# bwohlberg/sporco

Hardware: AMD Instinct MI355X
Metric: ConvBPDN ADMM iterations/s (higher is better)
Workload: dtype f32; 1 GPU; admm.cbpdn.ConvBPDN 512x512 greyscale, K=64 8x8 filters, N=32 images per GPU, lambda=0.05, default options (AutoRho, stats every iteration); global_images=32, parallelism=image-shard x1

## Files before the change

### include/sporco_amd.h

```cpp
#ifndef SPORCO_AMD_H
#define SPORCO_AMD_H

#include <stddef.h>
#include <stdint.h>

#ifdef __cplusplus
extern "C" {
#endif

#define SPORCO_AMD_F32 0
#define SPORCO_AMD_F64 1

#define SPORCO_AMD_OK 0
#define SPORCO_AMD_EINVAL (-1)
#define SPORCO_AMD_EHIP (-2)
#define SPORCO_AMD_ENOMEM (-3)
#define SPORCO_AMD_ESTATE (-4)


const char *sporco_amd_version(void);
const char *sporco_amd_last_error(void);
int sporco_amd_device_count(int *count);
int sporco_amd_device_info(int device, char *name, size_t name_len, int *cu_count,
                           size_t *hbm_bytes);
// ... 34 lines not shown
#define SPORCO_AMD_VAR_DMU0 22
#define SPORCO_AMD_VAR_WML 23
#define SPORCO_AMD_VAR_WMS 24
#define SPORCO_AMD_VAR_DX 32
#define SPORCO_AMD_VAR_DXF 33
#define SPORCO_AMD_VAR_DYF 34
#define SPORCO_AMD_VAR_DXFPRV 35
#define SPORCO_AMD_VAR_DYFPRV 36
#define SPORCO_AMD_VAR_DVF 37
#define SPORCO_AMD_VAR_DGF 38
#define SPORCO_AMD_VAR_DT0 39
#define SPORCO_AMD_VAR_DT1 40
#define SPORCO_AMD_VAR_DT2 41
#define SPORCO_AMD_VAR_DSX 42
#define SPORCO_AMD_VAR_DSU 43
#define SPORCO_AMD_VAR_COUNT 44

int sporco_amd_csc_create(const sporco_amd_dims *dims, int device, void *stream,
                          sporco_amd_csc_t *out);
int sporco_amd_csc_create_mc(const sporco_amd_dims *dims, int32_t dict_channels, int device,
                             void *stream, sporco_amd_csc_t *out);
int sporco_amd_csc_create_volume(const sporco_amd_dims *dims, int32_t depth, int device, void *stream,
                                 sporco_amd_csc_t *out);
int sporco_amd_csc_destroy(sporco_amd_csc_t h);
int sporco_amd_csc_sync(sporco_amd_csc_t h);
int sporco_amd_csc_stream(sporco_amd_csc_t h, void **stream);
#define SPORCO_AMD_QUERY_FUSED_COLS 0
#define SPORCO_AMD_QUERY_FUSED_ROWS 1
#define SPORCO_AMD_QUERY_FUSED_PGM 2
#define SPORCO_AMD_QUERY_DEVICE_FILTERS 3
#define SPORCO_AMD_QUERY_VFORM_LIVE 4
#define SPORCO_AMD_QUERY_PERSIST_RUNS 5
#define SPORCO_AMD_QUERY_CCMOD_GROUPS 6
int sporco_amd_csc_query(sporco_amd_csc_t h, int what, int *out);
int sporco_amd_csc_placement_report(sporco_amd_csc_t h, char *buf, size_t cap);
#define SPORCO_AMD_HINT_KEEP_VFORM 0
#define SPORCO_AMD_HINT_ONE_LAUNCH 1
#define SPORCO_AMD_MODE_COMPLEX_PAIR 2
#define SPORCO_AMD_VOLUME_FILTER_DEPTH 3
int sporco_amd_csc_set_hint(sporco_amd_csc_t h, int what, int value);

int sporco_amd_csc_set_signal(sporco_amd_csc_t h, const void *S);

int sporco_amd_csc_set_dict(sporco_amd_csc_t h, const void *D, int32_t dH, int32_t dW);
int sporco_amd_csc_set_dict_imag(sporco_amd_csc_t h, const void *D_imag, int32_t dH, int32_t dW);

int sporco_amd_csc_set_l1_weight(sporco_amd_csc_t h, const void *w, const int64_t shape[5]);
int sporco_amd_csc_set_l21_weight(sporco_amd_csc_t h, const void *w, const int64_t shape[5]);
int sporco_amd_csc_set_grad_weight(sporco_amd_csc_t h, const void *w);
int sporco_amd_csc_set_filter_sizes(sporco_amd_csc_t h, const int32_t *fh, const int32_t *fw);
int sporco_amd_csc_set_ams_mask(sporco_amd_csc_t h, const void *w, const int64_t shape[5]);

int sporco_amd_csc_upload(sporco_amd_csc_t h, int var, const void *src);
int sporco_amd_csc_download(sporco_amd_csc_t h, int var, void *dst);
int sporco_amd_csc_device_ptr(sporco_amd_csc_t h, int var, void **ptr_dev);


#define SPORCO_AMD_FLAG_NONNEG (1u << 0)
#define SPORCO_AMD_FLAG_NOBNDRY (1u << 1)
#define SPORCO_AMD_FLAG_JOINT (1u << 2)
#define SPORCO_AMD_FLAG_RESID (1u << 3)
#define SPORCO_AMD_FLAG_OBJ (1u << 4)
#define SPORCO_AMD_FLAG_XRRS (1u << 5)
#define SPORCO_AMD_FLAG_GEVAL_Y (1u << 6)
#define SPORCO_AMD_FLAG_FEVAL_Y (1u << 7)
#define SPORCO_AMD_FLAG_KEEP_X (1u << 8)
// ... 238 lines not shown
```

### sporco_amd/_lib.py

```python

import ctypes
import os

import numpy as np

F32, F64 = 0, 1

VAR_Y, VAR_U, VAR_X, VAR_XF, VAR_DF, VAR_SF = 0, 1, 2, 3, 4, 5
VAR_YF, VAR_XFPRV, VAR_YFPRV, VAR_VF, VAR_GF, VAR_AX, VAR_YPREV = 6, 7, 8, 9, 10, 11, 12
VAR_T0, VAR_T1, VAR_T2, VAR_ZF = 13, 14, 15, 16
VAR_CX, VAR_CU = 17, 18
VAR_MY0, VAR_MU0 = 19, 20
VAR_DMY0, VAR_DMU0 = 21, 22
VAR_WML, VAR_WMS = 23, 24
VAR_DX, VAR_DXF, VAR_DYF, VAR_DXFPRV, VAR_DYFPRV = 32, 33, 34, 35, 36
VAR_DVF, VAR_DGF, VAR_DT0, VAR_DT1, VAR_DT2 = 37, 38, 39, 40, 41
VAR_DSX, VAR_DSU = 42, 43
DSTEP_ISM, DSTEP_CG = 0, 1

FLAG_NONNEG = 1 << 0
FLAG_NOBNDRY = 1 << 1
FLAG_JOINT = 1 << 2
FLAG_RESID = 1 << 3
FLAG_OBJ = 1 << 4
FLAG_XRRS = 1 << 5
FLAG_GEVAL_Y = 1 << 6
FLAG_FEVAL_Y = 1 << 7
FLAG_KEEP_X = 1 << 8
FLAG_NO_X = 1 << 9
FLAG_GRADREG = 1 << 10
FLAG_AMS = 1 << 11
FLAG_DMASK = 1 << 12
QUERY_FUSED_COLS, QUERY_FUSED_ROWS, QUERY_FUSED_PGM, QUERY_DEVICE_FILTERS, QUERY_VFORM_LIVE = 0, 1, 2, 3, 4
QUERY_PERSIST_RUNS = 5
QUERY_CCMOD_GROUPS = 6
HINT_KEEP_VFORM = 0
HINT_ONE_LAUNCH = 1
MODE_COMPLEX_PAIR = 2
VOLUME_FILTER_DEPTH = 3

OUT_R2, OUT_S2, OUT_AX2, OUT_Y2, OUT_U2 = 0, 1, 2, 3, 4
OUT_DFID, OUT_L1, OUT_L21 = 5, 6, 7
OUT_XRRS_D2, OUT_XRRS_AX2, OUT_XRRS_B2 = 8, 9, 10
OUT_RGR = 11
OUT_CNSTR = 12
OUT_CGIT, OUT_CGN = 13, 14
OUT_COUNT = 16

PGM_F, PGM_DFID, PGM_L1, PGM_HESS, PGM_RSDL, PGM_FY, PGM_LIN, PGM_DXY2 = range(8)

EXPORTS = (
    'sporco_amd_version', 'sporco_amd_last_error', 'sporco_amd_device_count',
    'sporco_amd_device_info', 'sporco_amd_csc_create', 'sporco_amd_csc_create_mc', 'sporco_amd_csc_create_volume',
    'sporco_amd_csc_destroy',
    'sporco_amd_csc_sync', 'sporco_amd_csc_stream', 'sporco_amd_csc_query', 'sporco_amd_csc_placement_report', 'sporco_amd_csc_set_hint', 'sporco_amd_csc_set_signal', 'sporco_amd_csc_set_dict', 'sporco_amd_csc_set_dict_imag',
    'sporco_amd_csc_set_l1_weight', 'sporco_amd_csc_set_l21_weight',
    'sporco_amd_csc_set_grad_weight', 'sporco_amd_csc_set_ams_mask',
    'sporco_amd_csc_upload', 'sporco_amd_csc_download', 'sporco_amd_csc_device_ptr',
    'sporco_amd_csc_admm_iter', 'sporco_amd_csc_admm_iter_dev', 'sporco_amd_csc_admm_run',
    'sporco_amd_csc_admm_xstep', 'sporco_amd_csc_admm_relax',
    'sporco_amd_csc_admm_ystep', 'sporco_amd_csc_admm_ustep',
    'sporco_amd_csc_admm_stats', 'sporco_amd_csc_scale_u',
    'sporco_amd_csc_reconstruct', 'sporco_amd_csc_dhs_absmax',
    'sporco_amd_csc_pgm_grad', 'sporco_amd_csc_pgm_eval', 'sporco_amd_csc_pgm_prox_step',
    'sporco_amd_csc_pgm_iter', 'sporco_amd_csc_pgm_commit',
    'sporco_amd_csc_lincomb', 'sporco_amd_csc_pair_stats', 'sporco_amd_csc_copy',
    'sporco_amd_csc_pgm_resid', 'sporco_amd_csc_pgm_resid_stats',
    'sporco_amd_csc_fft_var', 'sporco_amd_csc_ifft_var',
# ... 768 lines not shown
```

### sporco_amd/csrc/api_admm_run.inc

```
    bool admm_run_supported(const sporco_amd_admm_params &p) const {
        return !cplx && std::is_same<T, float>::value && rows_ok && mr_ok(p) && (fused || fused_slabs) && !fused_mc &&
               !tail_mode && !(p.flags & (F_XRRS | F_GRADREG | F_KEEP_X | F_FEVAL_Y)) &&
               (!(p.flags & F_JOINT) || joint_rows_ok(p)) && p.lmbda >= 0.0 && p.rho > 0.0 &&
               !std::getenv("SPORCO_AMD_HOST_LOOP");
    }

    bool persist_ok(const sporco_amd_admm_params &p, const sporco_amd_admm_ctrl &c, bool vf,
                    bool has_reduce) const {
        const bool off = sw.persist >= 0 ? sw.persist != 1 : !hint_one_launch;
        return !off && vf && !has_reduce && fused && !fused_slabs && Ks == K && run_always_emit &&
               admm_persist_supported<T>(H, W, K) && !wl1.ptr && c.max_iter >= 3 &&
               !(p.flags & (F_NOBNDRY | F_AMS | F_JOINT)) && admm_persist_resident<T>(H, W, K, CN);
    }
    PersistIterArgs<T> persist_iter_args(const sporco_amd_admm_params &p, const T *vin, T *vout,
                                         double *prow, double *pcol) {
        PersistIterArgs<T> a;
        cx<T> *Xf = cv(SPORCO_AMD_VAR_XF);
        a.fwd.y = a.fwd.u = nullptr;
        a.fwd.v = vin;
        a.fwd.flags = p.flags;
        a.fwd.C = C;
        a.fwd.N = N;
        a.fwd.dH = p.dH;
        a.fwd.dW = p.dW;
// ... 65 lines not shown
            pst_grid = grid;
        }
        AdmmPersistArgs<T> a;
        const int p0 = index0 & 1;
        a.iter[p0] = persist_iter_args(p, v_prev, v_other, part_rows, part_f);
        a.iter[p0 ^ 1] = persist_iter_args(p, v_other, v_prev, pst_part_rows, pst_part_f);
        a.blk = static_cast<PersistIterArgs<T> *>(pst_blk);
        a.ctl_blk = pst_ctl;
        a.ctl = ctl_dev;
        a.rec = reinterpret_cast<AdmmRecord *>(rec_ring) + index0;
        a.index0 = index0;
        a.max_iter = max_iter - index0;
        a.bar = pst_bar;
        a.n_row_tiles = (int)nrow;
        a.n_col_tiles = (int)ncol;
        a.want_dfid = (p.flags & F_OBJ) ? 1 : 0;
        a.want_sums = want_sums ? 1 : 0;
        a.dfid_scale = 1.0 / ((double)H * W);
        SA_HIP(hipMemsetAsync(pst_bar, 0, sizeof(unsigned) * kPersistBarWords, st));
        {
            ProfScope ps(prof, PS_PERSIST);
            launch_admm_persist<T>(st, a, grid);
        }
        unsigned bar[16];
        SA_HIP(hipMemcpyAsync(bar, pst_bar, sizeof(bar), hipMemcpyDeviceToHost, st));
        sync();
        if (bar[2]) throw Error(SPORCO_AMD_EHIP, "one-launch solve: a grid barrier did not complete");
        xf_tiled = true;
        ++pst_runs;
        return (int)bar[3];
    }

    int64_t enqueue_iter_ctl(const sporco_amd_admm_params &p, const T *vin = nullptr,
                             T *vout = nullptr) {
        T *Y = vin ? nullptr : static_cast<T *>(vars[SPORCO_AMD_VAR_Y]);
        T *U = vin ? nullptr : static_cast<T *>(vars[SPORCO_AMD_VAR_U]);
        cx<T> *Xf = cv(SPORCO_AMD_VAR_XF);
        {
            RowsFwdArgs<T> ra;
            ra.y = Y;
            ra.u = U;
            ra.v = vin;
            ra.flags = p.flags;
            ra.C = C;
            ra.N = N;
            if (vin) {
                ra.wl1 = wl1;
                ra.dH = p.dH;
                ra.dW = p.dW;
                ra.ams_bits = ams_bits_of(p);
                ra.ams_k = Ku - 1;
            }
            ra.s2 = T(1);
            ra.t = Xf;
            ra.Ks = Ks;
            ra.twA = twRows;
            ra.H = H;
            ra.W = W;
            ra.CN = CN;
            ra.K = K;
            ra.P = P;
            ra.ctl = ctl_dev;
            ProfScope ps(prof, vin ? PS_ROWS_FWD_V : PS_ROWS_FWD);
            launch_rows_fwd<T>(st, ra);
        }
        {
            FusedColsArgs<T> fa;
// ... 37 lines not shown
        pa.twW = planW.tw<T>();
        pa.y = Y;
        pa.u = U;
        pa.y_out = y_alt;
        pa.u_out = u_alt;
        pa.v_in = vin;
        pa.v_out = vout;
        pa.x = nullptr;
        pa.scale = T(1.0 / ((double)H * (double)W));
        pa.rlx = (T)p.rlx;
        pa.thr = T(0);
        pa.u_scale = T(1);
        pa.flags = p.flags;
        pa.H = H;
        pa.W = W;
        pa.C = C;
        pa.N = N;
        pa.K = K;
        pa.dH = p.dH;
        pa.dW = p.dW;
        pa.P = P;
        pa.wl1 = wl1;
        pa.Ks = Ks;
        pa.ams_bits = ams_bits_of(p);
        pa.ams_k = Ku - 1;
        pa.partials = part_rows;
        pa.ctl = ctl_dev;
        int64_t nt = 0;
        if (!run_always_emit) {
            ProfScope ps(prof, vin ? PS_ROWS_INV_POST_V : PS_ROWS_INV_POST);
            nt = launch_rows_inv_post<T>(st, pa);
        }
        pa.t_next = Xf;
        {
            ProfScope ps(prof, vin ? PS_ROWS_INV_POST_V_EMIT : PS_ROWS_INV_POST_EMIT);
            nt = launch_rows_inv_post<T>(st, pa);
        }
        if (!vout) {
            std::swap(vars[SPORCO_AMD_VAR_Y], reinterpret_cast<void *&>(y_alt));
            std::swap(vars[SPORCO_AMD_VAR_U], reinterpret_cast<void *&>(u_alt));
        }
        return nt;
    }

    int admm_run(const sporco_amd_admm_params &p, const sporco_amd_admm_ctrl &c,
                 sporco_amd_admm_record *records, double *rho_out, double *u_scale_out,
                 sporco_amd_reduce_fn reduce, void *user) override {
        require_ready();
        if (!admm_run_supported(p)) return -1;
        if (gv_live) ensure_yu();
        SA_REQUIRE(c.max_iter >= 0, "max_iter must not be negative");
        if (c.max_iter == 0) {
            *rho_out = p.rho;
            *u_scale_out = p.u_scale;
            return 0;
        }
        if (!y_alt) alloc_alt_pair();
        const bool nn = p.flags & F_NONNEG, jn = p.flags & F_JOINT;
        if (v_live && (!vform_ok(p) || !vform_same_opts(p))) ensure_yu();
        const bool vf = vform_ok(p) && (v_live || c.max_iter >= 4 || hint_vform);
        if (!vf) ensure_yu();
        const bool v_at_entry = v_live;
        T *const v_entry = v_cur;
        const T v_entry_thr = v_thr, v_entry_thr21 = v_thr21;
        if (!ctl_dev) SA_HIP(hipMalloc((void **)&ctl_dev, sizeof(AdmmCtl)));
        if (rec_cap < c.max_iter) {
// ... 17 lines not shown
        in.xi = c.rho_xi;
        in.mu21 = p.mu;
        in.k = c.k0;
        in.stable_run = stable_run;
        in.emitted = t_ready ? 1 : 0;
        in.is_f32 = 1;
        in.autorho = c.auto_rho;
        in.period = c.period > 0 ? c.period : 1;
        in.autoscaling = c.auto_scaling;
        in.stdres = c.std_residuals;
        in.need_resid = c.need_residuals;
        in.thr_prev = v_at_entry ? (float)v_entry_thr : 0.f;
        in.thr21_prev = v_at_entry ? (float)v_entry_thr21 : 0.f;
        in.no_speculation = sw.no_speculation ? 1 : 0;
        run_always_emit = !in.no_speculation && E <= ((int64_t)1 << 22);
        if (run_always_emit) in.no_speculation = 2;
        launch_admm_ctl_init(st, ctl_dev, in);
        SA_HIP(hipMemsetAsync(out_dev, 0, sizeof(double) * kOutSlots, st));
        const int ahead = c.lookahead > 0 ? c.lookahead : 3;
        int enq = 0, done = 0, stop_at = -1;
        int lag = std::getenv("SPORCO_AMD_RUN_LAG") ? std::atoi(std::getenv("SPORCO_AMD_RUN_LAG")) : 0;
        auto poll = [&](int upto, bool block) {
            while (done < upto && stop_at < 0) {
                if (rec_ring[done].seq != done + 1) {
                    if (!block) return;
                    if (hipStreamQuery(st) == hipSuccess && rec_ring[done].seq != done + 1)
                        throw Error(SPORCO_AMD_EHIP, "device-driven solve: record not written");
                    continue;
                }
                if (rec_ring[done].stop) stop_at = done;
                ++done;
            }
        };
        T *vb_in = v_at_entry ? v_entry : nullptr;
        T *const vb_first = vf ? (vb_in == y_alt ? u_alt : y_alt) : nullptr;
        auto enqueue_one = [&]() {
            T *vb_out = vf ? (vb_in == y_alt ? u_alt : y_alt) : nullptr;
            const int64_t nt = enqueue_iter_ctl(p, vb_in, vb_out);
            vb_in = vb_out;
            if (want_sums) {
                const int slots[7] = {SPORCO_AMD_OUT_R2, SPORCO_AMD_OUT_S2, SPORCO_AMD_OUT_AX2,
                                      SPORCO_AMD_OUT_Y2, SPORCO_AMD_OUT_U2, SPORCO_AMD_OUT_L1,
                                      SPORCO_AMD_OUT_L21};
                const double scales[7] = {1, 1, 1, 1, 1, 1, 1};
                const int fslots[2] = {SPORCO_AMD_OUT_DFID, SPORCO_AMD_OUT_RGR};
                const double fscales[2] = {1.0 / ((double)H * W), 1.0 / ((double)H * W)};
                const bool dfid = p.flags & F_OBJ;
                {
                    ProfScope ps(prof, PS_FINALIZE);
                    launch_finalize2(st, part_rows, (int)nt, 8, (p.flags & F_JOINT) ? 7 : 6, slots,
                                     scales, part_f, part_f_rows,
                                     1, dfid ? 1 : 0, fslots, fscales, out_dev);
                }
                if (reduce) reduce(user, out_dev);
                else if (comm_user) comm_reduce_sums(comm_user, out_dev, st);
            }
            launch_admm_ctl_update(st, ctl_dev, out_dev, rec_ring + enq, enq, true);
            ++enq;
        };
        const bool shard = reduce != nullptr || comm_user != nullptr;
        const int wlag = shard ? 0 : lag;
        if (persist_ok(p, c, vf, shard)) {
            enqueue_one();
            T *v0 = vb_in, *v1 = (v0 == y_alt) ? u_alt : y_alt;
            enq += run_persist(p, 1, c.max_iter, v0, v1, want_sums);
            if (c.need_residuals) poll(enq, false);
        }
        for (; enq < c.max_iter && stop_at < 0 && !persist_ok(p, c, vf, shard);) {
            enqueue_one();
            if (c.need_residuals) {
                poll(enq - lag, false);
                if (stop_at < 0 && enq - wlag - done > ahead) poll(enq - wlag - ahead, true);
            }
        }
        if (shard && want_sums && c.need_residuals) {
            if (stop_at < 0) poll(enq, true);
            if (stop_at >= 0)
                while (enq < c.max_iter && enq < stop_at + 1 + ahead) enqueue_one();
        }
        sync();
        poll(enq, false);
        const int n = stop_at >= 0 ? stop_at + 1 : enq;
        if (!vf && ((enq - n) & 1)) {
            std::swap(vars[SPORCO_AMD_VAR_Y], reinterpret_cast<void *&>(y_alt));
            std::swap(vars[SPORCO_AMD_VAR_U], reinterpret_cast<void *&>(u_alt));
        }
        if (vf) {
            T *other_first = vb_first == y_alt ? u_alt : y_alt;
            v_cur = ((n - 1) & 1) ? other_first : vb_first;
            v_thr = (T)(p.lmbda / rec_ring[n - 1].rho);
            v_thr21 = (T)(p.mu / rec_ring[n - 1].rho);
            if (n >= 2) {
                v_prev_kind = 2;
// ... 104 lines not shown
```

### sporco_amd/csrc/csc_api.hip

```cpp
#include "csc_impl.h"

#include <chrono>
#include <string>

namespace sporco_amd {

thread_local std::string g_last_error;
std::atomic<int64_t> g_xfer[4];
const char *kProfNames[PS_COUNT] = {"fft_r2c_rows",     "fft_c2c_cols_fwd", "sm_solve",
                                           "fft_c2c_cols_inv", "fft_c2r_rows",     "admm_post",
                                           "fused_cols_sm",    "rows_fwd",         "rows_inv_post",
                                           "rows_inv_post_emit",
                                           "rows_fwd_v",       "rows_inv_post_v",  "rows_inv_post_v_emit",
                                           "pgm_grad_ifft",    "pgm_rows_prox",    "pgm_fft_momentum",
                                           "finalize",         "pgm_elementwise",  "other",
                                           "admm_persist_run",
                                    "setcoef_rows",     "setcoef_cols",     "ccmod_grad_tiled",
                                    "fft_c2r_vpost",    "fft_c2r_vpost_emit",
                                    "inhib_update"};

struct Switches {
    bool unfused, old_rows, no_pad, no_vform, no_speculation, no_cols_sm, md_generic, cns_generic, cg_host,
        placement_off, placement_force;
    int persist;
// ... 99 lines not shown
    }
    cx<T> *twRows = nullptr;
    double *part_rows = nullptr;
    double *pst_part_rows = nullptr, *pst_part_f = nullptr;
    void *pst_blk = nullptr;
    AdmmCtl *pst_ctl = nullptr;
    unsigned *pst_bar = nullptr;
    int pst_grid = 0, pst_runs = 0;
    T *y_alt = nullptr, *u_alt = nullptr;
    bool x_stale = false, x_invalid = false;
    bool md_x_pending = false;
    bool prev_in_alt = false;
    bool v_live = false;
    T *v_cur = nullptr;
    T v_thr = T(0), v_prev_thr = T(0);
    T v_thr21 = T(0), v_prev_thr21 = T(0), vp_thr21 = T(0);
    bool v_nonneg = false, v_joint = false;
    uint32_t v_opts = 0;
    int v_dH = 1, v_dW = 1;
    int v_prev_kind = 0;
    bool vp_pending = false;
    T *vp_buf = nullptr, *vp_free = nullptr;
    T vp_thr = T(0);
    bool vp_nonneg = false;
    uint64_t touch_epoch = 0, fused_epoch = ~(uint64_t)0;
    bool gv_live = false, gv_nonneg = false;
    T gv_thr = T(0);
    uint64_t gen_epoch = ~(uint64_t)0;
    bool t_ready = false;
    int stable_run = 0;
    AdmmCtl *ctl_dev = nullptr;
    AdmmRecord *rec_ring = nullptr;
    int rec_cap = 0;
    CgCtl *cg_dev = nullptr;
    CgPinned *cg_pin = nullptr;
    sporco_amd_admm_params last_p;
    bool zf_tiled = false;
    cx<T> *gpart = nullptr;
    int ccmod_groups = 1;
    bool pgm_tiled = false, pgm_x_stale = false;
    sporco_amd_pgm_params last_pgm;
    double *part_pgm = nullptr, *part_pgm2 = nullptr;
    cx<T> *ccmod_r = nullptr;
    cx<T> *pgm_ey = nullptr;
    bool pgm_held = false;
    bool run_always_emit = false;
    T *ghh = nullptr, *ghw = nullptr, *wg = nullptr;
    bool have_wg = false;
    T *g1t = nullptr;
    bool g1_valid = false;
    double g1_rho = 0.0, g1_mu = 0.0;

    int padded_filters(int H_, int W_, int K_) const {
        if (K_ % 2 == 0 || sw.unfused || sw.no_pad)
            return K_;
        const bool cols = fused_cols_supported<T>(H_, K_ + 1) || fused_slabs_supported<T>(H_, K_ + 1);
        return (cols && rows_supported<T>(W_, K_ + 1)) ? K_ + 1 : K_;
    }

    Csc(const sporco_amd_dims &d, int dev, void *stream, int cd, int depth_ = 1) : dm(d), device(dev) {
        SA_REQUIRE(d.H >= 1 && d.W >= 1 && d.C >= 1 && d.N >= 1 && d.K >= 1,
                   "all dimensions must be >= 1");
        SA_REQUIRE(cd == 1 || cd == d.C,
                   "a multi-channel dictionary needs as many channels as the signal");
        SA_HIP(hipSetDevice(device));
        H = d.H;
// ... 137 lines not shown
        (void)hipStreamSynchronize(st);
        place_release_spares();
        inhib_release();
        big_free(gemit);
        if (part_vpost) (void)hipFree(part_vpost);
        big_free(cols_out[0]);
        big_free(cols_out[1]);
        for (hipEvent_t e : place_ev)
            if (e) (void)hipEventDestroy(e);
        for (auto &v : vars) big_free(v);
        big_free(y_alt);
        big_free(u_alt);
        big_free(work);
        y_alt = u_alt = nullptr;
        work = nullptr;
        for (void *p : {(void *)pst_part_rows, (void *)pst_part_f, pst_blk, (void *)pst_ctl, (void *)pst_bar,
                        (void *)cns_w, (void *)cns_sft, (void *)flt_h, (void *)flt_w,
                        (void *)zf_ch, (void *)zfv_buf, (void *)md_sft, (void *)md_coef, (void *)pgm_rx[0], (void *)pgm_rx[1]})
            if (p) (void)hipFree(p);
        for (void *p : {(void *)dft, (void *)sft, (void *)gramt, (void *)part_f, (void *)twA, (void *)twB,
                        (void *)twRows, (void *)part_rows, (void *)y_alt, (void *)u_alt, (void *)part_pgm, (void *)part_pgm2, (void *)ccmod_r, (void *)pgm_ey, (void *)gpart,
                        (void *)qpart, (void *)coop_flags, (void *)ghh, (void *)ghw, (void *)wg, (void *)g1t, (void *)ism_gam, (void *)ism_del, (void *)ism_mm, (void *)dft_mc, (void *)sft_mc, (void *)bt_mc, (void *)cns_f, (void *)cns_m, (void *)sft_eff, (void *)coef_t, (void *)ams_bits, (void *)gramz_t,
                        (void *)cns_yold, (void *)md_s, (void *)dism_gam, (void *)dism_del, (void *)dism_mm,
                        (void *)dwork, (void *)pcn_stats, (void *)work, (void *)innerb, (void *)gram, (void *)dpad, (void *)sreal,
                        (void *)wl1_buf, (void *)wl21_buf, (void *)wams_buf, (void *)wdat_buf, (void *)part_a, (void *)part_b, (void *)part_cs, (void *)df_im, (void *)pgm_es[0], (void *)pgm_es[1], (void *)pgm_es[2], (void *)pgm_es[3],
                        (void *)out_dev_own})
            if (p) (void)hipFree(p);
        if (out_pinned) (void)hipHostFree(out_pinned);
        if (coop_err) (void)hipHostFree(coop_err);
        if (rec_ring) (void)hipHostFree(rec_ring);
        if (cg_pin) (void)hipHostFree((void *)cg_pin);
        if (cg_dev) (void)hipFree(cg_dev);
        if (ctl_dev) (void)hipFree(ctl_dev);
        planW.destroy();
        planH.destroy();
        if (depth > 1) planD.destroy();
        if (own_stream) (void)hipStreamDestroy(st);
    }

    int64_t KD() const { return (int64_t)Cd * K; }
    static bool var_is_signal_real(int var) {
        return var >= SPORCO_AMD_VAR_MY0 && var <= SPORCO_AMD_VAR_DMU0;
    }
    size_t var_bytes(int var) const {
        if (var == SPORCO_AMD_VAR_SF) return sizeof(cx<T>) * npix * CNs;
        if (var_is_signal_real(var)) return sizeof(T) * (int64_t)H * W * CNs;
        if (var_is_dict_sized(var))
            return var_is_complex(var) ? sizeof(cx<T>) * npix * KD()
                                       : sizeof(T) * (int64_t)H * W * KD();
        if (var == SPORCO_AMD_VAR_CX || var == SPORCO_AMD_VAR_CU) return sizeof(T) * E * Cd;
        return var_is_complex(var) ? sizeof(cx<T>) * EF : sizeof(T) * E;
    }

    size_t var_alloc_bytes(int var) const {
        return var == SPORCO_AMD_VAR_XF ? sizeof(cx<T>) * (size_t)std::max(EF, EFt) : var_bytes(var);
    }
    void *var_ptr(int var) {
        SA_REQUIRE(var_is_valid(var), "unknown state variable id");
        if (var == SPORCO_AMD_VAR_Y || var == SPORCO_AMD_VAR_U) {
            ++touch_epoch;
            if (v_live || gv_live) ensure_yu();
        }
        if (!vars[var]) {
            const size_t nb = var_alloc_bytes(var);
            big_alloc(&vars[var], nb);
            SA_HIP(hipMemsetAsync(vars[var], 0, nb, st));
// ... 52 lines not shown
    bool cols_striped() const { return cols_out[0] != nullptr; }
    void alloc_cols_out() {
        if (cols_out[0] || !std::is_same<T, float>::value || !fused || fused_slabs || tail_mode || Ks != K || !rows_ok || mr)
            return;
        const size_t plane = sizeof(cx<T>) * (size_t)CN * H * K;
        const size_t be = plane * (size_t)((Wf + 1) / 2), bo = plane * (size_t)(Wf / 2);
        if (!placement_on(be)) return;
        void *p0 = nullptr;
        big_alloc(&p0, be);
        cols_out[0] = static_cast<cx<T> *>(p0);
        cols_out[1] = static_cast<cx<T> *>(place_alloc(bo, {{p0, be}}, "cols_out_odd"));
    }
    void alloc_alt_pair() {
        if (y_alt) return;
        (void)var_ptr(SPORCO_AMD_VAR_XF);
        place_var(SPORCO_AMD_VAR_XF, {SPORCO_AMD_VAR_Y, SPORCO_AMD_VAR_U}, "T");
        void *t = vars[SPORCO_AMD_VAR_XF];
        const size_t tb = var_alloc_bytes(SPORCO_AMD_VAR_XF), nb = sizeof(T) * (size_t)E;
        y_alt = static_cast<T *>(place_alloc(nb, {{t, tb}}, "V0"));
        u_alt = static_cast<T *>(place_alloc(nb, {{t, tb}}, "V1"));
        place_var(SPORCO_AMD_VAR_Y, {SPORCO_AMD_VAR_XF}, "Y");
        place_var(SPORCO_AMD_VAR_U, {SPORCO_AMD_VAR_XF}, "U");
        alloc_cols_out();
        place_release_spares();
    }
    int query(int what) override {
        if (what == SPORCO_AMD_QUERY_FUSED_COLS) return (fused || fused_slabs || fused_mc) ? 1 : 0;
        if (what == SPORCO_AMD_QUERY_FUSED_ROWS) return rows_ok ? 1 : 0;
        if (what == SPORCO_AMD_QUERY_FUSED_PGM) return pgm_fused_ok() ? 1 : 0;
        if (what == SPORCO_AMD_QUERY_DEVICE_FILTERS) return K;
        if (what == SPORCO_AMD_QUERY_VFORM_LIVE) return (v_live || gv_live) ? 1 : 0;
        if (what == SPORCO_AMD_QUERY_PERSIST_RUNS) return pst_runs;
        if (what == SPORCO_AMD_QUERY_CCMOD_GROUPS) return ccmod_group_count();
        throw Error(SPORCO_AMD_EINVAL, "unknown query");
    }

#include "api_placement.inc"
#include "api_transforms.inc"
#include "api_setup.inc"
#include "api_admm_run.inc"
#include "api_admm.inc"
#include "api_pgm.inc"
#include "api_dictupdate.inc"
#include "api_consensus.inc"
#include "api_maskdcpl.inc"
#include "api_dstep.inc"
#include "api_inhib.inc"
};

CscBase *make_csc(const sporco_amd_dims &dims, int dict_channels, int device, void *stream, int depth) {
    if (dims.dtype == SPORCO_AMD_F32) return new Csc<float>(dims, device, stream, dict_channels, depth);
    if (dims.dtype == SPORCO_AMD_F64) return new Csc<double>(dims, device, stream, dict_channels, depth);
    throw Error(SPORCO_AMD_EINVAL, "dtype must be SPORCO_AMD_F32 or SPORCO_AMD_F64");
}

}
```

### sporco_amd/csrc/csc_rows.h

```cpp
#pragma once

#include "common.h"
#include "csc_fused.h"
#include "csc_kernels.h"

namespace sporco_amd {

template <typename T> struct RowsFwdArgs {
    const T *y, *u;
    T s2;
    cx<T> *t;
    const cx<T> *twA;
    int H, W, CN, K;
    int64_t P;
    const T *v = nullptr;
    T thr_prev = T(0);
    uint32_t flags = 0;
    T thr21_prev = T(0);
    int C = 1, N = 0;
    Weight<T> wl1;
    int dH = 1, dW = 1;
    const uint32_t *ams_bits = nullptr;
    int ams_k = -1;
    int y_bcast = 0;
    int Ks = 0;
    const AdmmCtl *ctl = nullptr;
    int persist = 0;
    int stagger_groups = 1, stagger_sleeps = 0;
};

template <typename T> struct RowsPostArgs {
    const cx<T> *t;
    const cx<T> *t_odd = nullptr;
    const cx<T> *twW;
    const cx<T> *twA;
    cx<T> *t_next;
    int emit_u = 0;
    const T *y, *u;
    T *y_out, *u_out;
    T *x;
    const T *v_in = nullptr;
    T *v_out = nullptr;
    T thr_prev = T(0);
    T thr21_prev = T(0);
    T scale;
    T rlx, thr, u_scale;
    T thr21 = T(0);
    uint32_t flags;
    int H, W, C, N, K, dH, dW;
    int64_t P;
    Weight<T> wl1;
    int Ks = 0;
    const uint32_t *ams_bits = nullptr;
    int ams_k = -1;
    double *partials;
    const AdmmCtl *ctl = nullptr;
    int persist = 0;
    int stagger_groups = 1, stagger_sleeps = 0;
};

template <typename T>
void launch_ams_pack(hipStream_t st, const Weight<T> &mask, uint32_t *bits, int H, int W, int C,
                     int N);

template <typename T> struct RowsProxArgs {
    const cx<T> *t_in;
    cx<T> *t_out;
    T *x;
    const cx<T> *twA, *twW;
    T scale, thr;
    uint32_t flags;
    int H, W, C, N, K, dH, dW;
    int64_t P;
    int Ks = 0;
    Weight<T> wl1;
    double *partials;
    int persist = 0;
    int stagger_groups = 1, stagger_sleeps = 0;
};
template <typename T> int64_t launch_rows_inv_prox_fwd(hipStream_t st, const RowsProxArgs<T> &a);

template <typename T> bool rows_joint_supported(int W, int C, int K);
template <typename T> bool rows_supported(int W, int K);
bool rows_mr_width(int W);
template <typename T> void rows_twiddles(int W, cx<T> *twA);
template <typename T> void launch_rows_fwd(hipStream_t st, const RowsFwdArgs<T> &a);
template <typename T> int64_t launch_rows_inv_post(hipStream_t st, const RowsPostArgs<T> &a);

template <typename T> struct PersistIterArgs {
    RowsFwdArgs<T> fwd;
    FusedColsArgs<T> cols;
// ... 22 lines not shown
```

### sporco_amd/csrc/csc_rows_body.inc

```
#include "csc_rows.h"

#include <cmath>
#include <cstdlib>

#include "csc_ctl_dev.h"
#include "csc_fused_body.h"
#include "regfft.h"

namespace sporco_amd {

namespace {

using namespace regfft;

struct alignas(16) cf2 {
    cf a, b;
};

constexpr int kN1 = 32;
constexpr size_t rows_lds_bytes(int NW) {
    return sizeof(f2) * 16 * NW * 64 + sizeof(double) * 8 * 16;
}

template <int N1, int NW> constexpr int spectral_waves() { return regfft::mr_length(N1) ? (N1 + 1) / 2 : NW; }
template <int N1, int NW> constexpr int spectral_lines() { return regfft::mr_length(N1) ? 2 : N1 / NW; }
template <int N1> __device__ __forceinline__ bool second_line(int w) { return (N1 & 1) == 0 || w != 0; }
template <int N1, int NW> __device__ __forceinline__ int line_of(int w, int j) {
    if (j == 0) return w;
    if (j == 1) return w == 0 ? N1 / 2 : N1 - w;
    if (j == 2) return w == 0 ? 8 : 16 - w;
    if (j == 3) return w == 0 ? 24 : 16 + w;
    if (j == 4) return 4 + w;
    if (j == 5) return 28 - w;
    if (j == 6) return 9 + w;
    return 23 - w;
}

__host__ __device__ constexpr bool first_half4(int k1) {
    return k1 < 4 || k1 == 8 || (k1 >= 13 && k1 <= 19) || k1 == 24 || k1 > 28;
}
__host__ __device__ constexpr int group_of(int N1, int NW, int k1) {
    if (NW == 4) return first_half4(k1) ? 0 : 1;
    return NW == 16 ? (k1 >= (N1 + 1) / 2 ? 1 : 0) : ((k1 < 8 || k1 == 16 || k1 > 24) ? 0 : 1);
}
__host__ __device__ constexpr int kl_of(int N1, int NW, int k1) {
    if (NW == 4) {
        int r = 0;
        for (int o = 0; o < k1; ++o) r += first_half4(o) == first_half4(k1) ? 1 : 0;
        return r;
    }
    if (NW == 16) return k1 >= (N1 + 1) / 2 ? k1 - (N1 + 1) / 2 : k1;
    if (group_of(N1, NW, k1) == 0) return k1 < 8 ? k1 : (k1 == 16 ? 8 : k1 - 16);
    return k1 < 16 ? k1 - 8 : k1 - 9;
}

__device__ __forceinline__ float soft1(float v, float thr) {
    float m = fabsf(v) - thr;
    m = m > 0.f ? m : 0.f;
    return __builtin_copysignf(m, v);
}
__device__ __forceinline__ float soft1_pos(float v, float thr) { return v - sa_med3(v, -thr, thr); }
template <int MODE> __device__ __forceinline__ float soft1_m(float v, float thr) {
    if constexpr (MODE == 1) return soft1(v, thr);
    else return soft1_pos(v, thr);
}

template <int NW, bool COH = false, int N1 = kN1>
__device__ __forceinline__ void spatial_to_spectral(cf (&v)[N1], const cf *twA, cf *t, int CN, int H,
                                                    int K, int cn, int k, int h, bool pv, int w,
                                                    int lane, f2 *L, int &token) {
    constexpr int J = spectral_lines<N1, NW>(), NA = spectral_waves<N1, NW>();
    constexpr int NG = 2;
    constexpr int LPG = J / NG;
    constexpr int LBW = ilog2(NW);
    const bool act = NA >= NW || w < NA;
    dif1<N1, false>(v, 0);
#pragma unroll
    for (int i = 1; i < N1; ++i) {
        cf tw;
        sa_uload2(reinterpret_cast<const float *>(twA + w * N1 + i), tw.re, tw.im);
        v[i] = cmul(v[i], tw);
    }
    reg_fence<N1>(v, 0, token);

    cf z[J * NW];
    static_for<NG>([&](auto gc) {
// ... 613 lines not shown
            if (WRITE_X) buf_store_cf(Xb, voff, soff, mk<float>(xs[0], xs[1]));
            if constexpr (EMIT_T && SF == 0) {
                v[n1] = mk<float>(emit_y * yn[0] - emit_s * un[0], emit_y * yn[1] - emit_s * un[1]);
            } else if constexpr (PARK && b * B >= NP) {
                f2 t;
                t.x = yn[0] - un[0];
                t.y = yn[1] - un[1];
                L[((n1 - NP) * NW + w) * 64 + lane] = t;
            } else if (EMIT_T) {
                v[n1] = mk<float>(yn[0] - un[0], yn[1] - un[1]);
            }
        }
    });
    if constexpr (PARK) {
#pragma unroll
        for (int i = 0; i < NP; ++i) {
            const f2 t = L[(i * NW + w) * 64 + lane];
            v[NP + i] = mk<float>(t.x, t.y);
        }
    }

    SA_VGPR_FENCE3(s_r2, s_s2, s_x2);
    SA_VGPR_FENCE3(s_y2, s_u2, s_l1);
    if (EMIT_T) {
        reg_fence<N1>(v, 0, token);
        spatial_to_spectral<NW, COH, N1>(v, a->twA, a->t_next, CN, a->H, a->Ks ? a->Ks : a->K, cn, k, h, pv, w, lane,
                                         L, token);
        __syncthreads();
    }

    double acc[8] = {(double)s_r2, (double)s_s2, (double)s_x2,   (double)s_y2,
                     (double)s_u2, (double)s_l1, (double)s_l21, 0.0};
    const int64_t tile = (int64_t)h * tiles_x + bx;
    block_sum_store<8, COH>(acc, scratch, a->partials + tile * 8);
}

template <int NW, bool WRITE_X, int MODE, bool EMIT_T, bool JOINT = false, int SF = 0, int N1 = kN1>
__global__ void __launch_bounds__(NW * 64, (JOINT && EMIT_T && NW == 8) ? 4 : 1)
rows_inv_post_kernel(const RowsPostArgs<float> a_in) {
    if (a_in.ctl && (a_in.ctl->stop | (a_in.ctl->emit != (EMIT_T ? 1 : 0)))) return;
    const int tiles_x = JOINT ? a_in.N * (a_in.K >> 5) : (int)((a_in.P + 127) / 128);
    rows_tile_loop(a_in, tiles_x, a_in.H, [tiles_x](auto a, int bx, int h) {
        rows_inv_post_tile<NW, WRITE_X, MODE, EMIT_T, JOINT, SF, false, N1>(a, bx, h, tiles_x);
    });
}

template <int NW, bool GENERAL, int N1 = kN1, typename AP>
__device__ __forceinline__ void rows_inv_prox_fwd_tile(AP ap, int bx, int h, int tiles_x) {
    constexpr int W = N1 * NW;
    const auto &a = *ap;
    const int tid = threadIdx.x;
    const int lane = tid & 63;
    const int w = sa_readfirstlane(tid >> 6);
    const int64_t p = (int64_t)bx * 128 + 2 * lane;
    const bool pv = p < a.P;
    const int CN = a.C * a.N;
    const int cn = pv ? (int)(p / a.K) : 0, k = pv ? (int)(p % a.K) : 0;
    f2 *L = dyn_lds<f2>();
    double *scratch = reinterpret_cast<double *>(L + 16 * NW * 64);
    int token = 0;

    cf v[N1];
    spectral_to_spatial<NW, false, N1>(v, a.twW, a.t_in, CN, a.H, a.Ks ? a.Ks : a.K, cn, k, h, pv, w, lane, L,
                                       token);

    const int64_t rowoff = (int64_t)h * W * a.P;
    const uint32_t rowbytes = (uint32_t)((int64_t)W * a.P * sizeof(float));
    const BufRsrc Xb = a.x ? make_rsrc(a.x + rowoff, rowbytes) : make_rsrc(a.t_in, 0u);
    const int voff = pv ? (int)(p * (int64_t)sizeof(float)) : (int)0x80000000;
    const int pixbytes = (int)(a.P * (int64_t)sizeof(float));
    const float scale = a.scale;
    const bool nonneg = a.flags & F_NONNEG, nob = a.flags & F_NOBNDRY;
    int wlane = 0;
    const int ws4 = (int)a.wl1.stride[4];
    if (GENERAL) {
        const int c = cn / a.N, n = cn % a.N;
        wlane = (int)(c * a.wl1.stride[2] + n * a.wl1.stride[3] + k * a.wl1.stride[4]);
// ... 41 lines not shown
        rows_inv_prox_fwd_tile<NW, GENERAL, N1>(a, bx, h, tiles_x);
    });
}


constexpr int kBarGroup0 = 16, kBarStride = 16;
__device__ __forceinline__ void grid_barrier(unsigned *bar, unsigned nblk) {
    sa_wait_stores();
    __syncthreads();
    if (threadIdx.x == 0 && sa_load_agent(bar + 2) == 0u) {
        const unsigned gen = sa_load_agent(bar + 1);
        const unsigned g = blockIdx.x & 7u, per = nblk >> 3;
        bool last = false;
        if ((sa_atomic_inc_agent(bar + kBarGroup0 + kBarStride * g) + 1u) % per == 0u)
            last = (sa_atomic_inc_agent(bar + kBarGroup0 + kBarStride * 8) + 1u) % 8u == 0u;
        if (last) {
            sa_store_agent(bar + 1, gen + 1);
        } else {
            int polls = 0;
            while (sa_load_agent(bar + 1) == gen) {
                sa_spin_pause();
                if (++polls > (1 << 22)) {
                    sa_store_agent(bar + 2, 1u);
                    break;
                }
            }
        }
    }
    __syncthreads();
}

__device__ __forceinline__ void persist_finalize(const double *prow, int nrow, const double *pcol, int ncol,
                                                 bool dfid, double dfid_scale, double *scratch, double *sums) {
    constexpr int FT = kFinalizeThreads;
    const int nv = 6 + (dfid ? 1 : 0);
    const int tid = threadIdx.x, nth = blockDim.x;
    if (tid < 16) sums[tid] = 0.0;
    for (int idx = tid; idx < nv * FT; idx += nth) {
        const int v = idx / FT, t = idx % FT;
        const double *p = v < 6 ? prow + v : pcol;
        const int n = v < 6 ? nrow : ncol, st = v < 6 ? 8 : 1;
        double s = 0.0;
        for (int b = t; b < n; b += FT) s = s + sa_load_agent(p + (int64_t)b * st);
        scratch[idx] = s;
    }
    __syncthreads();
    for (int w = FT / 2; w > 0; w >>= 1) {
        for (int idx = tid; idx < nv * w; idx += nth) {
            const int v = idx / w, t = idx % w;
            scratch[v * FT + t] = scratch[v * FT + t] + scratch[v * FT + t + w];
        }
        __syncthreads();
    }
    if (tid < nv) {
        const int slots[7] = {SPORCO_AMD_OUT_R2, SPORCO_AMD_OUT_S2, SPORCO_AMD_OUT_AX2, SPORCO_AMD_OUT_Y2,
                              SPORCO_AMD_OUT_U2, SPORCO_AMD_OUT_L1, SPORCO_AMD_OUT_DFID};
        sums[slots[tid]] = scratch[tid * FT] * (tid == 6 ? dfid_scale : 1.0);
    }
    __syncthreads();
}

template <int NW, int LP>
__global__ void __launch_bounds__(NW * 64) admm_persist_kernel(const AdmmPersistArgs<float> pa) {
    const int tid = threadIdx.x;
    const unsigned nblk = gridDim.x;
    AdmmCtl *c = pa.ctl_blk + blockIdx.x;
    double *scratch = dyn_lds<double>();
    double *sums = scratch + 7 * kFinalizeThreads;
    if (tid == 0) {
        *c = *pa.ctl;
        for (int par = 0; par < 2; ++par) {
            PersistIterArgs<float> *b = pa.blk + (size_t)par * nblk + blockIdx.x;
            *b = pa.iter[par];
            b->fwd.ctl = c;
            b->cols.ctl = c;
            b->post.ctl = c;
        }
    }
    sa_wait_stores();
    sa_scalar_cache_inv();
    __syncthreads();
    const int tiles_x = (int)((pa.iter[0].fwd.P + 127) / 128), H = pa.iter[0].fwd.H;
    const int64_t ntiles = (int64_t)tiles_x * H;
#ifdef SA_PERSIST_TIMING
    unsigned long long tl = sa_wall_clock(), tacc[8] = {0, 0, 0, 0, 0, 0, 0, 0};
#define SA_PT(i)                                   \
    {                                              \
        const unsigned long long t_ = sa_wall_clock(); \
        tacc[i] += t_ - tl;                        \
        tl = t_;                                   \
    }
#else
// ... 167 lines not shown
```

Measured before the change: 390.9 iterations/s (512x512, K=64, N=32 per GPU; summed over GPUs).

## Fold per-iteration sum reduction and ADMM control update into rows post kernel tail

Adds a last-block-done ticket to the emitting rows_inv_post kernel. The final block to finish reduces the per-tile partial sums and performs the ADMM control/record update in place, replacing the separate reduction and ctl-update launches for each iteration on the non-sharded path. This removes two or more kernel launches and their dependencies per iteration. In exchange every block pays an atomic and a store fence, and a single block now does the final reduction serially at the end of the kernel. The persist finalize is refactored to share the new reduction helper, which also gains a 4-way unrolled load loop.

After: 388.6 iterations/s (512x512, K=64, N=32 per GPU; summed over GPUs). Within noise of the previous version (-0.6%).

```diff
diff --git a/include/sporco_amd.h b/include/sporco_amd.h
--- a/include/sporco_amd.h
+++ b/include/sporco_amd.h
@@ -90,6 +90,7 @@
 #define SPORCO_AMD_QUERY_VFORM_LIVE 4
 #define SPORCO_AMD_QUERY_PERSIST_RUNS 5
 #define SPORCO_AMD_QUERY_CCMOD_GROUPS 6
+#define SPORCO_AMD_QUERY_LOOP_TAIL_RUNS 7
 int sporco_amd_csc_query(sporco_amd_csc_t h, int what, int *out);
 int sporco_amd_csc_placement_report(sporco_amd_csc_t h, char *buf, size_t cap);
 #define SPORCO_AMD_HINT_KEEP_VFORM 0
diff --git a/sporco_amd/_lib.py b/sporco_amd/_lib.py
--- a/sporco_amd/_lib.py
+++ b/sporco_amd/_lib.py
@@ -34,6 +34,7 @@
 QUERY_FUSED_COLS, QUERY_FUSED_ROWS, QUERY_FUSED_PGM, QUERY_DEVICE_FILTERS, QUERY_VFORM_LIVE = 0, 1, 2, 3, 4
 QUERY_PERSIST_RUNS = 5
 QUERY_CCMOD_GROUPS = 6
+QUERY_LOOP_TAIL_RUNS = 7
 HINT_KEEP_VFORM = 0
 HINT_ONE_LAUNCH = 1
 MODE_COMPLEX_PAIR = 2
diff --git a/sporco_amd/csrc/api_admm_run.inc b/sporco_amd/csrc/api_admm_run.inc
--- a/sporco_amd/csrc/api_admm_run.inc
+++ b/sporco_amd/csrc/api_admm_run.inc
@@ -121,7 +121,7 @@
     }
 
     int64_t enqueue_iter_ctl(const sporco_amd_admm_params &p, const T *vin = nullptr,
-                             T *vout = nullptr) {
+                             T *vout = nullptr, const RowsPostTail *tail = nullptr) {
         T *Y = vin ? nullptr : static_cast<T *>(vars[SPORCO_AMD_VAR_Y]);
         T *U = vin ? nullptr : static_cast<T *>(vars[SPORCO_AMD_VAR_U]);
         cx<T> *Xf = cv(SPORCO_AMD_VAR_XF);
@@ -225,6 +225,12 @@
             nt = launch_rows_inv_post<T>(st, pa);
         }
         pa.t_next = Xf;
+        if (tail) {
+            pa.tail = *tail;
+            pa.tail.ctl = ctl_dev;
+            pa.tail.part_f = part_f;
+            pa.tail.n_part_f = part_f_rows;
+        }
         {
             ProfScope ps(prof, vin ? PS_ROWS_INV_POST_V_EMIT : PS_ROWS_INV_POST_EMIT);
             nt = launch_rows_inv_post<T>(st, pa);
@@ -308,10 +314,30 @@
                 ++done;
             }
         };
+        const bool shard = reduce != nullptr || comm_user != nullptr;
+        const bool fold = !shard && !std::getenv("SPORCO_AMD_NO_LOOP_TAIL");
+        if (fold) {
+            if (!tail_ticket) SA_HIP(hipMalloc((void **)&tail_ticket, sizeof(unsigned)));
+            SA_HIP(hipMemsetAsync(tail_ticket, 0, sizeof(unsigned), st));
+            ++tail_runs;
+        }
         T *vb_in = v_at_entry ? v_entry : nullptr;
         T *const vb_first = vf ? (vb_in == y_alt ? u_alt : y_alt) : nullptr;
         auto enqueue_one = [&]() {
             T *vb_out = vf ? (vb_in == y_alt ? u_alt : y_alt) : nullptr;
+            if (fold) {
+                RowsPostTail tl;
+                tl.ticket = tail_ticket;
+                tl.rec = rec_ring + enq;
+                tl.index = enq;
+                tl.nv_rows = want_sums ? ((p.flags & F_JOINT) ? 7 : 6) : 0;
+                tl.want_dfid = (want_sums && (p.flags & F_OBJ)) ? 1 : 0;
+                tl.dfid_scale = 1.0 / ((double)H * W);
+                enqueue_iter_ctl(p, vb_in, vb_out, &tl);
+                vb_in = vb_out;
+                ++enq;
+                return;
+            }
             const int64_t nt = enqueue_iter_ctl(p, vb_in, vb_out);
             vb_in = vb_out;
             if (want_sums) {
@@ -334,7 +360,6 @@
             launch_admm_ctl_update(st, ctl_dev, out_dev, rec_ring + enq, enq, true);
             ++enq;
         };
-        const bool shard = reduce != nullptr || comm_user != nullptr;
         const int wlag = shard ? 0 : lag;
         if (persist_ok(p, c, vf, shard)) {
             enqueue_one();
diff --git a/sporco_amd/csrc/csc_api.hip b/sporco_amd/csrc/csc_api.hip
--- a/sporco_amd/csrc/csc_api.hip
+++ b/sporco_amd/csrc/csc_api.hip
@@ -155,6 +155,8 @@
     AdmmCtl *ctl_dev = nullptr;
     AdmmRecord *rec_ring = nullptr;
     int rec_cap = 0;
+    unsigned *tail_ticket = nullptr;
+    int tail_runs = 0;
     CgCtl *cg_dev = nullptr;
     CgPinned *cg_pin = nullptr;
     sporco_amd_admm_params last_p;
@@ -358,6 +360,7 @@
         if (cg_pin) (void)hipHostFree((void *)cg_pin);
         if (cg_dev) (void)hipFree(cg_dev);
         if (ctl_dev) (void)hipFree(ctl_dev);
+        if (tail_ticket) (void)hipFree(tail_ticket);
         planW.destroy();
         planH.destroy();
         if (depth > 1) planD.destroy();
@@ -476,6 +479,7 @@
         if (what == SPORCO_AMD_QUERY_VFORM_LIVE) return (v_live || gv_live) ? 1 : 0;
         if (what == SPORCO_AMD_QUERY_PERSIST_RUNS) return pst_runs;
         if (what == SPORCO_AMD_QUERY_CCMOD_GROUPS) return ccmod_group_count();
+        if (what == SPORCO_AMD_QUERY_LOOP_TAIL_RUNS) return tail_runs;
         throw Error(SPORCO_AMD_EINVAL, "unknown query");
     }
 
diff --git a/sporco_amd/csrc/csc_rows.h b/sporco_amd/csrc/csc_rows.h
--- a/sporco_amd/csrc/csc_rows.h
+++ b/sporco_amd/csrc/csc_rows.h
@@ -29,6 +29,17 @@
     int stagger_groups = 1, stagger_sleeps = 0;
 };
 
+struct RowsPostTail {
+    unsigned *ticket = nullptr;
+    AdmmCtl *ctl = nullptr;
+    AdmmRecord *rec = nullptr;
+    int index = 0;
+    int nv_rows = 0;
+    const double *part_f = nullptr;
+    int n_part_f = 0, want_dfid = 0;
+    double dfid_scale = 0.0;
+};
+
 template <typename T> struct RowsPostArgs {
     const cx<T> *t;
     const cx<T> *t_odd = nullptr;
@@ -57,6 +68,7 @@
     const AdmmCtl *ctl = nullptr;
     int persist = 0;
     int stagger_groups = 1, stagger_sleeps = 0;
+    RowsPostTail tail;
 };
 
 template <typename T>
diff --git a/sporco_amd/csrc/csc_rows_body.inc b/sporco_amd/csrc/csc_rows_body.inc
--- a/sporco_amd/csrc/csc_rows_body.inc
+++ b/sporco_amd/csrc/csc_rows_body.inc
@@ -52,6 +52,30 @@
     if (NW == 16) return k1 >= (N1 + 1) / 2 ? k1 - (N1 + 1) / 2 : k1;
     if (group_of(N1, NW, k1) == 0) return k1 < 8 ? k1 : (k1 == 16 ? 8 : k1 - 16);
     return k1 < 16 ? k1 - 8 : k1 - 9;
+}
+
+template <int NV>
+__device__ __forceinline__ void rows_sum_store(const double (&acc)[NV], double *scratch, double *dst, bool agent) {
+    const int lane = threadIdx.x & (kWave - 1);
+    const int wave = threadIdx.x / kWave;
+    const int nwave = (blockDim.x + kWave - 1) / kWave;
+    double w[NV];
+#pragma unroll
+    for (int i = 0; i < NV; ++i) w[i] = wave_sum(acc[i]);
+    if (lane == 0) {
+#pragma unroll
+        for (int i = 0; i < NV; ++i) scratch[wave * NV + i] = w[i];
+    }
+    __syncthreads();
+    if (threadIdx.x == 0) {
+#pragma unroll
+        for (int i = 0; i < NV; ++i) {
+            double s = 0.0;
+            for (int j = 0; j < nwave; ++j) s += scratch[j * NV + i];
+            if (agent) sa_store_agent(dst + i, s);
+            else dst[i] = s;
+        }
+    }
 }
 
 __device__ __forceinline__ float soft1(float v, float thr) {
@@ -731,17 +755,98 @@
     double acc[8] = {(double)s_r2, (double)s_s2, (double)s_x2,   (double)s_y2,
                      (double)s_u2, (double)s_l1, (double)s_l21, 0.0};
     const int64_t tile = (int64_t)h * tiles_x + bx;
-    block_sum_store<8, COH>(acc, scratch, a->partials + tile * 8);
+    rows_sum_store<8>(acc, scratch, a->partials + tile * 8, COH || (EMIT_T && a->tail.ticket != nullptr));
+}
+
+__device__ __forceinline__ void rows_finalize_sums(const double *prow, int nrow, int nv_rows, const double *pcol,
+                                                   int ncol, bool dfid, double dfid_scale, double *scratch,
+                                                   double *sums) {
+    constexpr int FT = kFinalizeThreads;
+    const int nv = nv_rows + (dfid ? 1 : 0);
+    const int tid = threadIdx.x, nth = blockDim.x;
+    if (tid < 16) sums[tid] = 0.0;
+    for (int idx = tid; idx < nv * FT; idx += nth) {
+        const int v = idx / FT, t = idx % FT;
+        const double *p = v < nv_rows ? prow + v : pcol;
+        const int n = v < nv_rows ? nrow : ncol;
+        const int64_t st = v < nv_rows ? 8 : 1;
+        double s = 0.0;
+        int b = t;
+        for (; b + 3 * FT < n; b += 4 * FT) {
+            const double v0 = sa_load_agent(p + (int64_t)b * st), v1 = sa_load_agent(p + (int64_t)(b + FT) * st);
+            const double v2 = sa_load_agent(p + (int64_t)(b + 2 * FT) * st),
+                         v3 = sa_load_agent(p + (int64_t)(b + 3 * FT) * st);
+            s = s + v0;
+            s = s + v1;
+            s = s + v2;
+            s = s + v3;
+        }
+        for (; b < n; b += FT) s = s + sa_load_agent(p + (int64_t)b * st);
+        scratch[idx] = s;
+    }
+    __syncthreads();
+    for (int w = FT / 2; w > 0; w >>= 1) {
+        for (int idx = tid; idx < nv * w; idx += nth) {
+            const int v = idx / w, t = idx % w;
+            scratch[v * FT + t] = scratch[v * FT + t] + scratch[v * FT + t + w];
+        }
+        __syncthreads();
+    }
+    if (tid < nv) {
+        const int slots[7] = {SPORCO_AMD_OUT_R2, SPORCO_AMD_OUT_S2, SPORCO_AMD_OUT_AX2, SPORCO_AMD_OUT_Y2,
+                              SPORCO_AMD_OUT_U2, SPORCO_AMD_OUT_L1, SPORCO_AMD_OUT_L21};
+        if (tid < nv_rows) sums[slots[tid]] = scratch[tid * FT] * 1.0;
+        else sums[SPORCO_AMD_OUT_DFID] = scratch[tid * FT] * dfid_scale;
+    }
+    __syncthreads();
+}
+
+template <typename A> __device__ __forceinline__ void rows_post_close(const A &a, int ntiles) {
+    double *scratch = dyn_lds<double>();
+    double *sums = scratch + 8 * kFinalizeThreads;
+    if (a.tail.nv_rows > 0) {
+        rows_finalize_sums(a.partials, ntiles, a.tail.nv_rows, a.tail.part_f, a.tail.n_part_f,
+                           a.tail.want_dfid != 0, a.tail.dfid_scale, scratch, sums);
+    } else {
+        if (threadIdx.x < 16) sums[threadIdx.x] = 0.0;
+        __syncthreads();
+    }
+    if (threadIdx.x == 0) {
+        admm_ctl_update_dev<float>(a.tail.ctl, sums, a.tail.rec, a.tail.index);
+        sa_store_agent(a.tail.ticket, 0u);
+    }
+}
+template <typename A> __device__ __forceinline__ void rows_post_tail(const A &a, int ntiles) {
+    double *scratch = dyn_lds<double>();
+    unsigned *last = reinterpret_cast<unsigned *>(scratch + 8 * kFinalizeThreads + 16);
+    __syncthreads();
+    if (threadIdx.x == 0) {
+        sa_wait_stores();
+        *last = (sa_atomic_inc_agent(a.tail.ticket) + 1u == gridDim.x) ? 1u : 0u;
+    }
+    __syncthreads();
+    if (*last) rows_post_close(a, ntiles);
 }
 
 template <int NW, bool WRITE_X, int MODE, bool EMIT_T, bool JOINT = false, int SF = 0, int N1 = kN1>
 __global__ void __launch_bounds__(NW * 64, (JOINT && EMIT_T && NW == 8) ? 4 : 1)
 rows_inv_post_kernel(const RowsPostArgs<float> a_in) {
-    if (a_in.ctl && (a_in.ctl->stop | (a_in.ctl->emit != (EMIT_T ? 1 : 0)))) return;
     const int tiles_x = JOINT ? a_in.N * (a_in.K >> 5) : (int)((a_in.P + 127) / 128);
+    if (a_in.ctl) {
+        if (a_in.ctl->stop) return;
+        if (a_in.ctl->emit != (EMIT_T ? 1 : 0)) {
+            if constexpr (EMIT_T) {
+                if (a_in.tail.ticket) rows_post_tail(a_in, tiles_x * a_in.H);
+            }
+            return;
+        }
+    }
     rows_tile_loop(a_in, tiles_x, a_in.H, [tiles_x](auto a, int bx, int h) {
         rows_inv_post_tile<NW, WRITE_X, MODE, EMIT_T, JOINT, SF, false, N1>(a, bx, h, tiles_x);
     });
+    if constexpr (EMIT_T) {
+        if (a_in.tail.ticket) rows_post_tail(a_in, tiles_x * a_in.H);
+    }
 }
 
 template <int NW, bool GENERAL, int N1 = kN1, typename AP>
@@ -849,32 +954,7 @@
 
 __device__ __forceinline__ void persist_finalize(const double *prow, int nrow, const double *pcol, int ncol,
                                                  bool dfid, double dfid_scale, double *scratch, double *sums) {
-    constexpr int FT = kFinalizeThreads;
-    const int nv = 6 + (dfid ? 1 : 0);
-    const int tid = threadIdx.x, nth = blockDim.x;
-    if (tid < 16) sums[tid] = 0.0;
-    for (int idx = tid; idx < nv * FT; idx += nth) {
-        const int v = idx / FT, t = idx % FT;
-        const double *p = v < 6 ? prow + v : pcol;
-        const int n = v < 6 ? nrow : ncol, st = v < 6 ? 8 : 1;
-        double s = 0.0;
-        for (int b = t; b < n; b += FT) s = s + sa_load_agent(p + (int64_t)b * st);
-        scratch[idx] = s;
-    }
-    __syncthreads();
-    for (int w = FT / 2; w > 0; w >>= 1) {
-        for (int idx = tid; idx < nv * w; idx += nth) {
-            const int v = idx / w, t = idx % w;
-            scratch[v * FT + t] = scratch[v * FT + t] + scratch[v * FT + t + w];
-        }
-        __syncthreads();
-    }
-    if (tid < nv) {
-        const int slots[7] = {SPORCO_AMD_OUT_R2, SPORCO_AMD_OUT_S2, SPORCO_AMD_OUT_AX2, SPORCO_AMD_OUT_Y2,
-                              SPORCO_AMD_OUT_U2, SPORCO_AMD_OUT_L1, SPORCO_AMD_OUT_DFID};
-        sums[slots[tid]] = scratch[tid * FT] * (tid == 6 ? dfid_scale : 1.0);
-    }
-    __syncthreads();
+    rows_finalize_sums(prow, nrow, 6, pcol, ncol, dfid, dfid_scale, scratch, sums);
 }
 
 template <int NW, int LP>
```
